# Oxel40/qtttgym

Hardware: AMD Instinct MI355X
Metric: env_steps_per_sec (higher is better)
Workload: dtype u64

## Files before the change

### qtttgym_amd/csrc/qttt_step_core.h

```cpp
#ifndef QTTT_STEP_CORE_H
#define QTTT_STEP_CORE_H
#include "qttt_state.h"

namespace {

struct StepPrep {
    u32 lo, hi, x16, pm, n6, mlo, mhi;
    u64 comps;
    bool legal, has_lo, cyc;
};

#define BITOP3(a, b, c, F) __builtin_amdgcn_bitop3_b32((a), (b), (c), (u32)([] { constexpr u32 A = 0xF0u, B = 0xCCu, C = 0xAAu; \
                                                                                 (void)A; (void)B; (void)C; return (F) & 0xFFu; }()))
template <u32 SH>
__device__ __forceinline__ u32 lshl_or(u32 a, u32 c) {
    u32 r;
    asm("v_lshl_or_b32 %0, %1, %2, %3" : "=v"(r) : "v"(a), "n"(SH), "v"(c));
    return r;
}

template <bool TRUSTED>
__device__ __forceinline__ StepPrep step_prep(u32 P1, u32 Q1, u32 act) {
    StepPrep s;
    const u32 a = act & 0xFFu, b = act >> 8;
    s.lo = TRUSTED ? a : min(a, b);
    s.hi = TRUSTED ? b : max(a, b);
    s.x16 = (a ^ b) << 16;
    const u32 pmS = ((1u << P1_CL_SHIFT) << (s.lo & 31u)) | ((1u << P1_CL_SHIFT) << (s.hi & 31u));
    s.legal = TRUSTED || (s.hi < 9u && s.lo != s.hi && (P1 & pmS) == 0u);
    s.pm = pmS >> P1_CL_SHIFT;
    s.n6 = P1 >> (P1_N_SHIFT - 2u);
    s.comps = (u64)Q1 | ((u64)((P1 >> P1_CHI_SHIFT) & 0xFu) << 32);
    s.mlo = (u32)(s.comps >> (s.lo & 63u)) & SLOT_LSB;
    s.mhi = (u32)(s.comps >> (s.hi & 63u)) & SLOT_LSB;
    asm("" : "+v"(s.mlo), "+v"(s.mhi));
    s.has_lo = s.mlo != 0u;
    s.cyc = (s.mlo & s.mhi) != 0u;
    return s;
}

__device__ __forceinline__ u32 step_child_end4(u32 lo, u32 hi, bool has_lo, bool cyc, u32 bit) {
    return ((!has_lo || (cyc && bit == 0u)) ? lo : hi) * 4u;
}

__device__ __forceinline__ u64 step_reroot(u64 P, u32 Q0, u32 x4, u32 n6) {
    u32 v4 = x4, prev4 = ~n6;
#pragma unroll
    for (int i = 0; i < 9; ++i) {
        const u32 t = (u32)(P >> v4);
        const u32 ec4 = t & 0x3Cu;
        P ^= (u64)((t ^ prev4) & 0x3Cu) << v4;
        if (ec4 == 0u) break;
        v4 ^= rotr32(Q0, ec4) & 0x3Cu;
        prev4 = ec4;
    }
    return P;
}

__device__ __forceinline__ void step_fields(const StepPrep &s, u32 &P1, u32 &Q0, u32 &Q1) {
    Q0 ^= rotr32(s.x16, s.n6 + 18u);
    const u32 c1 = (u32)(s.comps >> (ffbl_raw(s.mhi) & 63u)) & 0x1FFu;
    const u32 tsel = s.has_lo ? s.mlo : s.mhi;
    const u32 c32 = (u32)s.comps;
    const u32 y8 = (((c32 & 0x03FDFEFFu) + 0x03FDFEFFu) | c32) >> 8;
    const u32 sT = ffbl_raw(BITOP3(tsel, y8, SLOT_LSB, A | (~B & C)));
    const u64 ins = (u64)(s.pm | c1) << sT;
    const u32 q1 = c32 | (u32)ins;
    const u32 chi2 = (u32)(s.comps >> 32) | (u32)(ins >> 32);
    const u32 mpop = s.has_lo ? s.mhi : 0u;
    const u32 low = mpop - 1u;
    Q1 = BITOP3(q1, low, __builtin_amdgcn_alignbit(chi2, q1, 9u), (A & B) | (C & ~B));
    u32 p = P1 & ~((0xFu << P1_CHI_SHIFT) | (0xFu << P1_LX_SHIFT));
    p = lshl_or<P1_CHI_SHIFT>(mpop ? 0u : chi2, p);
    p = lshl_or<P1_CL_SHIFT>(s.cyc ? c1 : 0u, p);
    P1 = (p | s.x16) + (1u << P1_N_SHIFT);
}

__device__ __forceinline__ u32 step_line(u32 P0, u32 &P1, const uint8_t *lut) {
    const u32 par4 = P0 & 0x44444444u;
    const u32 even4 = lshl_or<8>(P1 & 4u, __builtin_amdgcn_udot8(par4, 0x00008421u, 0u, false) |
                                          (__builtin_amdgcn_udot8(par4, 0x84210000u, 0u, false) << 4));
    u32 cl4 = (P1 >> (P1_CL_SHIFT - 2u)) & 0x7FCu;
    asm("" : "+v"(cl4));
    const u32 pc = (u32)__builtin_popcount(cl4);
    u32 O4 = cl4 & ~even4;
    asm("" : "+v"(O4));
    const u32 X4 = pc >= 8u ? (O4 ^ 0x7FCu) : (cl4 & even4);
    const u32 win = *reinterpret_cast<const u32 *>(lut + X4) | *reinterpret_cast<const u32 *>(lut + O4);
    P1 = lshl_or<28>(BITOP3(win, pc, 8u, (A | B) & C), P1);
    return win;
}

__device__ __forceinline__ u32 step_line_xo(u32 P0, u32 &P1, const uint8_t *lut) {
    const u32 par4 = P0 & 0x44444444u;
    const u32 even4 = lshl_or<8>(P1 & 4u, __builtin_amdgcn_udot8(par4, 0x00008421u, 0u, false) |
                                          (__builtin_amdgcn_udot8(par4, 0x84210000u, 0u, false) << 4));
    u32 cl4 = (P1 >> (P1_CL_SHIFT - 2u)) & 0x7FCu;
    asm("" : "+v"(cl4));
    const u32 pc = (u32)__builtin_popcount(cl4);
    u32 O4 = cl4 & ~even4;
    asm("" : "+v"(O4));
    const u32 X4 = pc >= 8u ? (O4 ^ 0x7FCu) : (cl4 & even4);
    const u32 wx = *reinterpret_cast<const u32 *>(lut + X4), wo = *reinterpret_cast<const u32 *>(lut + O4);
    P1 = lshl_or<28>(BITOP3(wx | wo, pc, 8u, (A | B) & C), P1);
    return (wx & 1u) | ((wo & 1u) << 1);
}

__device__ __forceinline__ void step_auto_reset(u32 &P0, u32 &P1, u32 &Q0, u32 &Q1) {
    u32 gone = (u32)((int)P1 >> 31);
    asm("" : "+v"(gone));
    P0 &= ~gone;
    P1 &= ~gone;
    Q0 &= ~gone;
    Q1 &= ~gone;
}

template <bool AUTO_RESET, bool TRUSTED = false>
__device__ __forceinline__ u32 step_core(u32 &P0, u32 &P1, u32 &Q0, u32 &Q1, u32 act, u32 bit,
                                         const uint8_t *lut) {
    if (AUTO_RESET) {
        step_auto_reset(P0, P1, Q0, Q1);
    }
    const StepPrep s = step_prep<TRUSTED>(P1, Q1, act);
    if (s.legal) {
        const u64 P = step_reroot((u64)P0 | ((u64)P1 << 32), Q0, step_child_end4(s.lo, s.hi, s.has_lo, s.cyc, bit), s.n6);
        P0 = (u32)P;
        P1 = (u32)(P >> 32);
        step_fields(s, P1, Q0, Q1);
    }
    return step_line(P0, P1, lut);
}

__device__ __forceinline__ u32 step_core_both(u32 P0, u32 P1, u32 &Q0, u32 &Q1, u32 act, const uint8_t *lut,
                                              u32 &P0a, u32 &P1a, u32 &P0b, u32 &P1b, u32 &xo_a, u32 &xo_b) {
    const StepPrep s = step_prep<false>(P1, Q1, act);
    P0a = P0b = P0;
    P1a = P1b = P1;
    if (s.legal) {
        const u64 P = (u64)P0 | ((u64)P1 << 32);
        const u64 Pa = step_reroot(P, Q0, step_child_end4(s.lo, s.hi, s.has_lo, s.cyc, 0u), s.n6);
        const u64 Pb = s.cyc ? step_reroot(P, Q0, step_child_end4(s.lo, s.hi, s.has_lo, s.cyc, 1u), s.n6) : Pa;
        u32 F = P1;
        step_fields(s, F, Q0, Q1);
        F &= ~0x3Fu;
        P0a = (u32)Pa;
        P1a = F | ((u32)(Pa >> 32) & 0x3Fu);
        P0b = (u32)Pb;
        P1b = F | ((u32)(Pb >> 32) & 0x3Fu);
    }
    xo_a = step_line_xo(P0a, P1a, lut);
    xo_b = step_line_xo(P0b, P1b, lut);
    return s.legal ? (s.cyc ? 2u : 1u) : 0u;
}

}

#endif
```

### qtttgym_amd/csrc/qttt_step_kernels.h

```cpp
#ifndef QTTT_STEP_KERNELS_H
#define QTTT_STEP_KERNELS_H
#include "qttt_step_core.h"
#include "qttt_observation.h"

namespace {

template <bool DEVSTEP> struct StepKeySource {};
template <> struct StepKeySource<true> {
    const u32 *ctr;
    u64 seed;
};

template <int BLOCK, int BPL, bool HAS_BITS, bool AUTO_RESET, bool SAMPLE, bool OBS, bool DEVSTEP, bool OUT>
__device__ __forceinline__ void step_body(
    u64 *__restrict__ pP, u64 *__restrict__ pQ, uint16_t *__restrict__ actions,
    const uint8_t *__restrict__ bits, u32 key_fold, u32 key_hi, u32 id_base,
    u32 *__restrict__ reward_bits, uint8_t *__restrict__ terminated, ObsOut obs, int64_t i_begin,
    u32 last_groups, StepKeySource<DEVSTEP> sk) {
    constexpr u32 TILE_BOARDS = BLOCK * BPL;
    __shared__ __attribute__((aligned(16))) uint8_t lut[LINE_LUT_BYTES];
    constexpr bool ROWS = SAMPLE && BLOCK >= 512;
    constexpr u32 PT_WORDS = ROWS ? POLICY_ROWS_WORDS : POLICY_LUT_WORDS;
    constexpr int PRW = SAMPLE ? (int)((PT_WORDS + BLOCK - 1) / BLOCK) : 1;
    __shared__ __attribute__((aligned(16))) u32 prows[SAMPLE ? PT_WORDS : 1];
    __shared__ __attribute__((aligned(16))) uint8_t otile[OBS ? obs_lds_bytes(TILE_BOARDS) : 16];
    __shared__ __attribute__((aligned(16))) u32 olut[OBS ? OBS_LUT_BYTES / 4 : 4];
#ifdef QTTT_DEBUG_STAMPS
    const u64 st0 = __builtin_amdgcn_s_memrealtime();
#endif
    typedef Vec<u64, BPL> V64;
    typedef Vec<u32, BPL> V32;
    typedef Vec<uint16_t, BPL> V16;
    typedef Vec<uint8_t, BPL> V8;
    if constexpr (DEVSTEP) {
        const u64 key = launch_key(sk.seed, key_hi + *sk.ctr);
        key_fold ^= (u32)key;
        key_hi = (u32)(key >> 32);
    }
    const int64_t jb = (int64_t)blockIdx.x * BLOCK;
    const int64_t ib = i_begin + jb * BPL;
    const u32 ng = blockIdx.x + 1u == gridDim.x ? last_groups : (u32)BLOCK;
    const bool active = threadIdx.x < ng;
    const u32 g = active ? threadIdx.x : 0u;
    u32 olw = 0;
    if (OBS && threadIdx.x < OBS_LUT_BYTES / 4) olw = (&g_obs_lut.sel[0][0])[threadIdx.x];
    u32 prw[PRW];
    if (SAMPLE) {
#pragma unroll
        for (int k = 0; k < PRW; ++k) {
            const u32 w = threadIdx.x + (u32)k * BLOCK;
            const u32 *src = ROWS ? reinterpret_cast<const u32 *>(&g_policy_rows) : reinterpret_cast<const u32 *>(&g_policy_lut);
            prw[k] = w < PT_WORDS ? src[w] : 0u;
        }
    }
    V64 p = load_stream(&reinterpret_cast<const V64 *>(pP + ib)[g]);
    V64 q = load_stream(&reinterpret_cast<const V64 *>(pQ + ib)[g]);
    V16 act;
    V8 bt;
    if (!SAMPLE) act = load_stream(&reinterpret_cast<const V16 *>(actions + ib)[g]);
    if (HAS_BITS) bt = load_stream(&reinterpret_cast<const V8 *>(bits + ib)[g]);
    fill_line_lut_nosync<BLOCK>(lut);
    if (OBS && threadIdx.x < OBS_LUT_BYTES / 4) olut[threadIdx.x] = olw;
    if (SAMPLE) {
#pragma unroll
        for (int k = 0; k < PRW; ++k) {
            const u32 w = threadIdx.x + (u32)k * BLOCK;
            if (w < PT_WORDS) prows[w] = prw[k];
        }
    }
    ObsTiles T;
    if (OBS) T = obs_tiles<TILE_BOARDS>(otile, obs, ib);
    const u32 id0 = id_base + ((u32)jb + g) * BPL;
    u32 hbit[BPL], hpol[BPL];
#pragma unroll
    for (int k = 0; k < BPL; ++k) {
        hbit[k] = hpol[k] = 0u;
        if (SAMPLE) {
            const u32 h1 = lowbias32((id0 + (u32)k) ^ key_fold);
            hpol[k] = lowbias32(h1 ^ key_hi);
            hbit[k] = h1 >> 31;
            asm volatile("" : "+v"(hbit[k]), "+v"(hpol[k]));
        } else if (!HAS_BITS) {
            hbit[k] = collapse_bit_of((id0 + (u32)k) ^ key_fold);
            asm volatile("" : "+v"(hbit[k]));
        }
    }
    __syncthreads();
#ifdef QTTT_DEBUG_STAMPS
    asm volatile("s_waitcnt vmcnt(0)" ::: "memory");
    const u64 st1 = __builtin_amdgcn_s_memrealtime();
#endif
    if (active) {
        V32 rw;
        V8 tm;
#pragma unroll
        for (int k = 0; k < BPL; ++k) {
            u32 P0 = (u32)p.v[k], P1 = (u32)(p.v[k] >> 32);
            u32 Q0 = (u32)q.v[k], Q1 = (u32)(q.v[k] >> 32);
            u32 bit, av, win;
            if (SAMPLE) {
                const u32 h2 = hpol[k];
                bit = hbit[k];
                if (AUTO_RESET) {
                    step_auto_reset(P0, P1, Q0, Q1);
                    const u32 empty = ~(P1 >> P1_CL_SHIFT) & 0x1FFu;
                    av = ROWS ? policy_action_rows(prows, empty, h2) : policy_action(reinterpret_cast<const uint8_t *>(prows), empty, h2);
                    win = step_core<false, true>(P0, P1, Q0, Q1, av, bit, lut);
                } else {
                    const u32 empty = ~(P1 >> P1_CL_SHIFT) & 0x1FFu;
                    av = !(empty & (empty - 1u)) ? 0u : ROWS ? policy_action_rows(prows, empty, h2)
                                                             : policy_action(reinterpret_cast<const uint8_t *>(prows), empty, h2);
                    win = step_core<false>(P0, P1, Q0, Q1, av, bit, lut);
                }
                act.v[k] = (uint16_t)av;
            } else {
                av = act.v[k];
                if (HAS_BITS) bit = bt.v[k] & 1u;
                else bit = hbit[k];
                win = step_core<AUTO_RESET>(P0, P1, Q0, Q1, av, bit, lut);
            }
            p.v[k] = (u64)P0 | ((u64)P1 << 32);
            q.v[k] = (u64)Q0 | ((u64)Q1 << 32);
            if (OUT) {
                rw.v[k] = 0x80000000u | (win << 23);
                tm.v[k] = (uint8_t)(P1 >> 31);
            }
            if (OBS) obs_board(P0, P1, Q0, T, g * BPL + (u32)k, olut);
        }
        store_stream_sbase(pP + ib, g * (u32)sizeof(V64), p);
        store_stream_sbase(pQ + ib, g * (u32)sizeof(V64), q);
        if (SAMPLE && actions) store_stream(&reinterpret_cast<V16 *>(actions + ib)[g], act);
        if (OUT) {
            store_stream(&reinterpret_cast<V32 *>(reward_bits + ib)[g], rw);
            store_stream(&reinterpret_cast<V8 *>(terminated + ib)[g], tm);
        }
    }
    if (OBS) {
        const u32 ph = obs_all_phases(obs, ib, 15u);
        if ((ph & 3u) == 0u) {
            const u32 w0 = (threadIdx.x & ~63u) * BPL;
            __builtin_amdgcn_fence(__ATOMIC_ACQ_REL, "wavefront");
            __builtin_amdgcn_wave_barrier();
            if (w0 < ng * BPL) {
                if (ph == 0u) obs_wave_copy_out<TILE_BOARDS, true>(otile, obs, ib, w0, min(w0 + 64u * BPL, ng * BPL));
                else obs_wave_copy_out<TILE_BOARDS, false>(otile, obs, ib, w0, min(w0 + 64u * BPL, ng * BPL));
            }
        } else {
            __syncthreads();
            obs_copy_out<BLOCK, TILE_BOARDS>(otile, obs, ib, ng * BPL);
        }
    }
#ifdef QTTT_DEBUG_STAMPS
    const u64 st2 = __builtin_amdgcn_s_memrealtime();
    asm volatile("s_waitcnt vmcnt(0)" ::: "memory");
    const u64 st3 = __builtin_amdgcn_s_memrealtime();
    if (g_debug_stamps && (threadIdx.x & 63) == 0) {
        u64 *o = g_debug_stamps + ((int64_t)blockIdx.x * (BLOCK / 64) + (threadIdx.x >> 6)) * 4;
        o[0] = st0; o[1] = st1; o[2] = st2; o[3] = st3;
    }
#endif
}

template <int BLOCK, int BPL, bool HAS_BITS, bool AUTO_RESET, bool SAMPLE = false, bool OBS = false, bool DEVSTEP = false>
__global__ __launch_bounds__(BLOCK) void step_kernel(
    u64 *__restrict__ pP, u64 *__restrict__ pQ, uint16_t *__restrict__ actions,
    const uint8_t *__restrict__ bits, u32 key_fold, u32 key_hi, u32 id_base,
    u32 *__restrict__ reward_bits, uint8_t *__restrict__ terminated, ObsOut obs, int64_t i_begin,
    u32 last_groups, StepKeySource<DEVSTEP> sk) {
    step_body<BLOCK, BPL, HAS_BITS, AUTO_RESET, SAMPLE, OBS, DEVSTEP, true>(
        pP, pQ, actions, bits, key_fold, key_hi, id_base, reward_bits, terminated, obs, i_begin, last_groups, sk);
}

template <int BLOCK, int BPL, bool HAS_BITS, bool AUTO_RESET>
__global__ __launch_bounds__(BLOCK) void step_quiet_kernel(
    u64 *__restrict__ pP, u64 *__restrict__ pQ, const uint16_t *__restrict__ actions,
    const uint8_t *__restrict__ bits, u32 key_fold, u32 id_base, int64_t i_begin, u32 last_groups) {
    step_body<BLOCK, BPL, HAS_BITS, AUTO_RESET, false, false, false, false>(
        pP, pQ, const_cast<uint16_t *>(actions), bits, key_fold, 0u, id_base, nullptr, nullptr,
        ObsOut{nullptr, nullptr, nullptr, nullptr, nullptr, nullptr}, i_begin, last_groups, StepKeySource<false>{});
}

constexpr int FUSED_MAX_PLIES = 64;
struct FusedKeys { u64 k[FUSED_MAX_PLIES]; };
constexpr int FUSED_OUT_NONE = 0, FUSED_OUT_LAST = 1, FUSED_OUT_EVERY = 2;
template <bool HAS_BITS, bool AUTO_RESET, int OUT>
__global__ __launch_bounds__(QTTT_BLOCK) void step_fused_kernel(
    u64 *__restrict__ pP, u64 *__restrict__ pQ, const uint16_t *__restrict__ actions,
    const uint8_t *__restrict__ bits, FusedKeys keys, u32 id_hi_fold, u32 id_base,
    u32 *__restrict__ reward_bits, uint8_t *__restrict__ terminated, int64_t out_stride, int64_t n,
    int32_t n_steps) {
    static_assert(OUT == FUSED_OUT_EVERY, "the output-free forms are the overload below");
    __shared__ __attribute__((aligned(16))) uint8_t lut[LINE_LUT_BYTES];
    const int64_t ib = (int64_t)blockIdx.x * QTTT_BLOCK;
    const int64_t i = ib + threadIdx.x;
    const int64_t il = i < n ? i : 0;
    const u64 P = load_stream(&pP[il]), Q = load_stream(&pQ[il]);
    fill_line_lut<QTTT_BLOCK>(lut);
    if (i >= n) return;
    u32 P0 = (u32)P, P1 = (u32)(P >> 32), Q0 = (u32)Q, Q1 = (u32)(Q >> 32);
    const u32 id = (id_base + (u32)i) ^ id_hi_fold;
    const uint16_t *a_blk = actions + ib;
    const uint8_t *b_blk = HAS_BITS ? bits + ib : nullptr;
    const u32 lane = threadIdx.x;
    u32 win = 0;
    u64 key = keys.k[0];
    u32 *r_blk = reward_bits + ib;
    uint8_t *t_blk = terminated + ib;
    u32 act = load_stream(&a_blk[lane]), bit_in = HAS_BITS ? (u32)load_stream(&b_blk[lane]) : 0u;
    for (int32_t t = 0; t < n_steps; ++t) {
        const u64 key_next = keys.k[(t + 1) & (FUSED_MAX_PLIES - 1)];
        const bool more = t + 1 < n_steps;
        a_blk += more ? n : 0;
        if (HAS_BITS) b_blk += more ? n : 0;
        const u32 act_next = load_stream(&a_blk[lane]), bit_next = HAS_BITS ? (u32)load_stream(&b_blk[lane]) : 0u;
        const u32 bit = HAS_BITS ? (bit_in & 1u) : collapse_bit_of(id ^ (u32)key);
        win = step_core<AUTO_RESET>(P0, P1, Q0, Q1, act, bit, lut);
        if (out_stride != 0 || t == n_steps - 1) {
            store_stream(&r_blk[lane], 0x80000000u | (win << 23));
            store_stream(&t_blk[lane], (uint8_t)(P1 >> 31));
        }
        r_blk += out_stride;
        t_blk += out_stride;
        key = key_next;
        act = act_next;
        bit_in = bit_next;
    }
    store_stream(&pP[i], (u64)P0 | ((u64)P1 << 32));
    store_stream(&pQ[i], (u64)Q0 | ((u64)Q1 << 32));
}

constexpr int FUSED_PREFETCH = 2;
constexpr int RESIDENT_MAX_PLIES = 256;
constexpr int RESIDENT_BLOCK = QTTT_BLOCK;
template <int CAP>
struct ResidentKeys { u64 k[CAP]; };
template <bool HAS_BITS, bool AUTO_RESET, int OUT, int CAP, int BLOCK>
__global__ __launch_bounds__(BLOCK) void step_fused_kernel(
    u64 *__restrict__ pP, u64 *__restrict__ pQ, const uint16_t *__restrict__ actions,
    const uint8_t *__restrict__ bits, ResidentKeys<CAP> keys, u32 id_hi_fold, u32 id_base,
    u32 *__restrict__ reward_bits, uint8_t *__restrict__ terminated, int64_t n, int32_t n_steps) {
    static_assert(OUT == FUSED_OUT_LAST || OUT == FUSED_OUT_NONE, "every ply's outputs: the kernel above");
    static_assert(sizeof(ResidentKeys<CAP>) + 64 + 256 <= 4096, "4 KB of kernel arguments, the hidden ones included");
    __shared__ __attribute__((aligned(16))) uint8_t lut[LINE_LUT_BYTES];
    const int64_t ib = (int64_t)blockIdx.x * BLOCK;
    const int64_t i = ib + threadIdx.x;
    const int64_t il = i < n ? i : 0;
    const u64 P = load_stream(&pP[il]), Q = load_stream(&pQ[il]);
    fill_line_lut<BLOCK>(lut);
    if (i >= n) return;
    u32 P0 = (u32)P, P1 = (u32)(P >> 32), Q0 = (u32)Q, Q1 = (u32)(Q >> 32);
    const u32 id = (id_base + (u32)i) ^ id_hi_fold;
    const uint16_t *a_blk = actions + ib;
    const uint8_t *b_blk = HAS_BITS ? bits + ib : nullptr;
    const u32 lane = threadIdx.x;
    u32 win = 0;
    u64 key = keys.k[0];
    u32 act[FUSED_PREFETCH], bit_in[FUSED_PREFETCH];
#pragma unroll
    for (int k = 0; k < FUSED_PREFETCH; ++k) {
        if (k > 0) {
            const bool more = k < n_steps;
            a_blk += more ? n : 0;
            if (HAS_BITS) b_blk += more ? n : 0;
        }
        act[k] = load_stream(&a_blk[lane]);
        bit_in[k] = HAS_BITS ? (u32)load_stream(&b_blk[lane]) : 0u;
    }
    asm volatile("" : "+v"(P0), "+v"(P1), "+v"(Q0), "+v"(Q1));
    for (int32_t t = 0; t < n_steps; ++t) {
        const u64 key_next = keys.k[(CAP & (CAP - 1)) == 0 ? (t + 1) & (CAP - 1) : t + 1 < CAP ? t + 1 : 0];
        const bool more = t + FUSED_PREFETCH < n_steps;
        a_blk += more ? n : 0;
        if (HAS_BITS) b_blk += more ? n : 0;
        const u32 act_far = load_stream(&a_blk[lane]), bit_far = HAS_BITS ? (u32)load_stream(&b_blk[lane]) : 0u;
        const u32 bit = HAS_BITS ? (bit_in[0] & 1u) : collapse_bit_of(id ^ (u32)key);
        win = step_core<AUTO_RESET>(P0, P1, Q0, Q1, act[0], bit, lut);
        key = key_next;
#pragma unroll
        for (int k = 0; k + 1 < FUSED_PREFETCH; ++k) {
            act[k] = act[k + 1];
            bit_in[k] = bit_in[k + 1];
        }
        act[FUSED_PREFETCH - 1] = act_far;
        bit_in[FUSED_PREFETCH - 1] = bit_far;
    }
    if constexpr (OUT == FUSED_OUT_LAST) {
        store_stream(&reward_bits[i], 0x80000000u | (win << 23));
        store_stream(&terminated[i], (uint8_t)(P1 >> 31));
    }
    store_stream(&pP[i], (u64)P0 | ((u64)P1 << 32));
    store_stream(&pQ[i], (u64)Q0 | ((u64)Q1 << 32));
}

template <int BLOCK, bool AUTO_RESET, bool RETURNS = false, bool KEEP = false>
__global__ __launch_bounds__(BLOCK) void step_random_fused_kernel(
    u64 *__restrict__ pP, u64 *__restrict__ pQ, FusedKeys keys, u64 board_offset,
    uint16_t *__restrict__ actions_out, u32 *__restrict__ reward_bits, uint8_t *__restrict__ terminated,
    int64_t out_stride, int64_t n, int32_t n_steps, float *__restrict__ returns) {
    __shared__ __attribute__((aligned(16))) uint8_t lut[LINE_LUT_BYTES];
    __shared__ __attribute__((aligned(16))) uint8_t plut[POLICY_LUT_WORDS * 4];
    __shared__ uint8_t nth9[NTH9_BYTES];
    const int64_t ib = (int64_t)blockIdx.x * BLOCK;
    const int64_t i = ib + threadIdx.x;
    const bool active = i < n;
    const int64_t il = active ? i : 0;
    const u64 P = load_stream(&pP[il]), Q = load_stream(&pQ[il]);
    fill_policy_lut<BLOCK>(plut);
    fill_nth9<BLOCK>(nth9);
    fill_line_lut<BLOCK>(lut);
    if (!active) return;
    u32 P0 = (u32)P, P1 = (u32)(P >> 32), Q0 = (u32)Q, Q1 = (u32)(Q >> 32);
    const u32 id = fold_id(board_offset + (u64)i);
    uint16_t *a_blk = actions_out ? actions_out + ib : nullptr;
    u32 *r_blk = reward_bits ? reward_bits + ib : nullptr;
    uint8_t *t_blk = terminated ? terminated + ib : nullptr;
    const int64_t a_step = actions_out ? out_stride : 0, r_step = reward_bits ? out_stride : 0;
    const u32 lane = threadIdx.x;
    u32 lines = 0;
    u64 key = keys.k[0];
    asm volatile("" : "+v"(P0), "+v"(P1), "+v"(Q0), "+v"(Q1));
    for (int32_t t = 0; t < n_steps; ++t) {
        const u64 key_next = keys.k[(t + 1) & (FUSED_MAX_PLIES - 1)];
        const u32 h1 = lowbias32(id ^ (u32)key);
        const u32 h2 = lowbias32(h1 ^ (u32)(key >> 32));
        u32 act, win;
        if (AUTO_RESET) {
            step_auto_reset(P0, P1, Q0, Q1);
            const u32 empty = ~(P1 >> P1_CL_SHIFT) & 0x1FFu;
            act = policy_action_nth9(plut, nth9, empty, h2);
            win = step_core<false, true>(P0, P1, Q0, Q1, act, h1 >> 31, lut);
        } else {
            const u32 empty = ~(P1 >> P1_CL_SHIFT) & 0x1FFu;
            act = (empty & (empty - 1u)) ? policy_action_nth9(plut, nth9, empty, h2) : 0u;
            win = step_core<false, false>(P0, P1, Q0, Q1, act, h1 >> 31, lut);
        }
        if (KEEP || out_stride != 0 || t == n_steps - 1) {
            if (KEEP || a_blk) store_stream_sbase_word<2>(a_blk, lane * 2u, act);
            if (KEEP || r_blk) {
                store_stream_sbase_word<4>(r_blk, lane * 4u, 0x80000000u | (win << 23));
                store_stream_sbase_word<1>(t_blk, lane, P1 >> 31);
            }
        }
        if (RETURNS) lines += win & 1u;
        a_blk += a_step;
        r_blk += r_step;
        t_blk += r_step;
        key = key_next;
    }
    if (RETURNS) returns[i] -= (float)lines;
    store_stream(&pP[i], (u64)P0 | ((u64)P1 << 32));
    store_stream(&pQ[i], (u64)Q0 | ((u64)Q1 << 32));
}

}

#endif
```

Measured before the change: 342.3 billion.

## Keep board state unpacked in registers across fused step loop

Introduces a ResidentBoard that splits the packed P1 word into separate registers (chance bits, cycle mask, done flag) for the whole multi-step loop, packing back only at the end. The per-ply step now avoids repeated mask/shift extraction and reinsertion, and uses SDWA min/max/xor to decode the action bytes. The legality test is folded into a single compare. This trades extra live registers for fewer ALU ops per step, and the rewritten legality and done-flag logic risks subtle semantic differences.

```diff
diff --git a/qtttgym_amd/csrc/qttt_step_core.h b/qtttgym_amd/csrc/qttt_step_core.h
--- a/qtttgym_amd/csrc/qttt_step_core.h
+++ b/qtttgym_amd/csrc/qttt_step_core.h
@@ -131,6 +131,91 @@
     return step_line(P0, P1, lut);
 }
 
+template <bool AUTO_RESET>
+struct ResidentBoard {
+    u32 P0, P1, Q0, Q1, H, CL, gone, wx, wo;
+
+    __device__ __forceinline__ void unpack(u32 p0, u32 p1, u32 q0, u32 q1) {
+        P0 = p0, Q0 = q0, Q1 = q1;
+        wx = wo = 0u;
+        gone = (u32)((int)p1 >> 31);
+        H = (p1 >> P1_CHI_SHIFT) & 0xFu;
+        CL = p1 & (0x1FFu << P1_CL_SHIFT);
+        P1 = p1 & ~((0xFu << P1_CHI_SHIFT) | (0x1FFu << P1_CL_SHIFT) | P1_DONE);
+        asm volatile("" : "+v"(P0), "+v"(P1), "+v"(Q0), "+v"(Q1), "+v"(H), "+v"(CL), "+v"(gone));
+    }
+
+    __device__ __forceinline__ void pack(u32 &p0, u32 &p1, u32 &q0, u32 &q1, u32 &win) const {
+        p0 = P0, q0 = Q0, q1 = Q1;
+        p1 = P1 | (H << P1_CHI_SHIFT) | CL | (gone & P1_DONE);
+        win = wx | wo;
+    }
+
+    __device__ __forceinline__ void ply(u32 act, u32 bit, const uint8_t *lut) {
+        if (AUTO_RESET) {
+            u32 g = gone;
+            asm("" : "+v"(g));
+            P0 &= ~g;
+            P1 &= ~g;
+            Q0 &= ~g;
+            Q1 &= ~g;
+            H &= ~g;
+            CL &= ~g;
+        }
+        StepPrep s;
+        asm("v_min_u32_sdwa %0, %1, %1 dst_sel:DWORD dst_unused:UNUSED_PAD src0_sel:BYTE_0 src1_sel:BYTE_1" : "=v"(s.lo) : "v"(act));
+        asm("v_max_u32_sdwa %0, %1, %1 dst_sel:DWORD dst_unused:UNUSED_PAD src0_sel:BYTE_0 src1_sel:BYTE_1" : "=v"(s.hi) : "v"(act));
+        asm("v_xor_b32_sdwa %0, %1, %1 dst_sel:WORD_1 dst_unused:UNUSED_PAD src0_sel:BYTE_0 src1_sel:BYTE_1" : "=v"(s.x16) : "v"(act));
+        const u32 cl_bit0 = 1u << P1_CL_SHIFT;
+        u32 pmS;
+        asm("v_lshl_or_b32 %0, %1, %2, %3" : "=v"(pmS) : "v"(cl_bit0), "v"(s.lo), "v"(cl_bit0 << (s.hi & 31u)));
+        const u32 z = CL & pmS;
+        s.pm = pmS >> P1_CL_SHIFT;
+        s.legal = s.hi < 9u && s.x16 > z;
+        s.n6 = P1 >> (P1_N_SHIFT - 2u);
+        s.comps = (u64)Q1 | ((u64)H << 32);
+        s.mlo = (u32)(s.comps >> (s.lo & 63u)) & SLOT_LSB;
+        s.mhi = (u32)(s.comps >> (s.hi & 63u)) & SLOT_LSB;
+        asm("" : "+v"(s.mlo), "+v"(s.mhi));
+        s.has_lo = s.mlo != 0u;
+        s.cyc = (s.mlo & s.mhi) != 0u;
+        if (s.legal) {
+            const u64 P = step_reroot((u64)P0 | ((u64)P1 << 32), Q0, step_child_end4(s.lo, s.hi, s.has_lo, s.cyc, bit), s.n6);
+            P0 = (u32)P;
+            P1 = (u32)(P >> 32);
+            Q0 ^= rotr32(s.x16, s.n6 + 18u);
+            const u32 c1 = (u32)(s.comps >> (ffbl_raw(s.mhi) & 63u)) & 0x1FFu;
+            const u32 tsel = s.has_lo ? s.mlo : s.mhi;
+            const u32 c32 = (u32)s.comps;
+            const u32 y8 = (((c32 & 0x03FDFEFFu) + 0x03FDFEFFu) | c32) >> 8;
+            const u32 sT = ffbl_raw(BITOP3(tsel, y8, SLOT_LSB, A | (~B & C)));
+            const u64 ins = (u64)(s.pm | c1) << sT;
+            const u32 q1 = c32 | (u32)ins;
+            const u32 chi2 = (u32)(s.comps >> 32) | (u32)(ins >> 32);
+            const u32 mpop = s.has_lo ? s.mhi : 0u;
+            const u32 low = mpop - 1u;
+            Q1 = BITOP3(q1, low, __builtin_amdgcn_alignbit(chi2, q1, 9u), (A & B) | (C & ~B));
+            H = mpop ? 0u : chi2;
+            CL = lshl_or<P1_CL_SHIFT>(s.cyc ? c1 : 0u, CL);
+            P1 = BITOP3(P1, ~(0xFu << P1_LX_SHIFT), s.x16, (A & B) | C) + (1u << P1_N_SHIFT);
+        }
+        const u32 par4 = P0 & 0x44444444u;
+        const u32 even4 = lshl_or<8>(P1 & 4u, __builtin_amdgcn_udot8(par4, 0x00008421u, 0u, false) |
+                                              (__builtin_amdgcn_udot8(par4, 0x84210000u, 0u, false) << 4));
+        u32 cl4 = CL >> (P1_CL_SHIFT - 2u);
+        asm("" : "+v"(cl4));
+        const u32 pc = (u32)__builtin_popcount(cl4);
+        u32 O4 = cl4 & ~even4;
+        asm("" : "+v"(O4));
+        const u32 X4 = pc >= 8u ? (O4 ^ 0x7FCu) : (cl4 & even4);
+        wx = *reinterpret_cast<const u32 *>(lut + X4);
+        wo = *reinterpret_cast<const u32 *>(lut + O4);
+        u32 nw = (u32)__builtin_amdgcn_sbfe(BITOP3(wx, wo, pc, A | B | C), 3u, 1u);
+        asm("" : "+v"(nw));
+        gone = AUTO_RESET ? nw : (gone | nw);
+    }
+};
+
 __device__ __forceinline__ u32 step_core_both(u32 P0, u32 P1, u32 &Q0, u32 &Q1, u32 act, const uint8_t *lut,
                                               u32 &P0a, u32 &P1a, u32 &P0b, u32 &P1b, u32 &xo_a, u32 &xo_b) {
     const StepPrep s = step_prep<false>(P1, Q1, act);
diff --git a/qtttgym_amd/csrc/qttt_step_kernels.h b/qtttgym_amd/csrc/qttt_step_kernels.h
--- a/qtttgym_amd/csrc/qttt_step_kernels.h
+++ b/qtttgym_amd/csrc/qttt_step_kernels.h
@@ -266,7 +266,8 @@
         act[k] = load_stream(&a_blk[lane]);
         bit_in[k] = HAS_BITS ? (u32)load_stream(&b_blk[lane]) : 0u;
     }
-    asm volatile("" : "+v"(P0), "+v"(P1), "+v"(Q0), "+v"(Q1));
+    ResidentBoard<AUTO_RESET> board;
+    board.unpack(P0, P1, Q0, Q1);
     for (int32_t t = 0; t < n_steps; ++t) {
         const u64 key_next = keys.k[(CAP & (CAP - 1)) == 0 ? (t + 1) & (CAP - 1) : t + 1 < CAP ? t + 1 : 0];
         const bool more = t + FUSED_PREFETCH < n_steps;
@@ -274,7 +275,7 @@
         if (HAS_BITS) b_blk += more ? n : 0;
         const u32 act_far = load_stream(&a_blk[lane]), bit_far = HAS_BITS ? (u32)load_stream(&b_blk[lane]) : 0u;
         const u32 bit = HAS_BITS ? (bit_in[0] & 1u) : collapse_bit_of(id ^ (u32)key);
-        win = step_core<AUTO_RESET>(P0, P1, Q0, Q1, act[0], bit, lut);
+        board.ply(act[0], bit, lut);
         key = key_next;
 #pragma unroll
         for (int k = 0; k + 1 < FUSED_PREFETCH; ++k) {
@@ -284,6 +285,7 @@
         act[FUSED_PREFETCH - 1] = act_far;
         bit_in[FUSED_PREFETCH - 1] = bit_far;
     }
+    board.pack(P0, P1, Q0, Q1, win);
     if constexpr (OUT == FUSED_OUT_LAST) {
         store_stream(&reward_bits[i], 0x80000000u | (win << 23));
         store_stream(&terminated[i], (uint8_t)(P1 >> 31));
```

Measured after the change: 361.9 billion, median of 6. 5.7% higher.
